# hangxu0304/DeepReduce

Measured on NVIDIA H100. Metric: ResNet-50 images/sec (whole job, device-timed, max over ranks), higher is better.
Workload: dtype bf16

## Files before the change

deepreduce_b200/ops/csrc/binding.cpp:

```cpp
#include <ATen/cuda/CUDAContext.h>
#include <c10/cuda/CUDAGuard.h>
#include <c10/cuda/CUDAStream.h>
#include <torch/extension.h>

#include <condition_variable>
#include <deque>
#include <mutex>
#include <thread>

#include "ops.h"

namespace py = pybind11;
using dr::EngineParams;

#define CHECK_CUDA_T(x) TORCH_CHECK((x).is_cuda() && (x).is_contiguous(), #x " must be a contiguous CUDA tensor")

static cudaStream_t cur_stream() { return at::cuda::getCurrentCUDAStream().stream(); }

static void check_last(const char* what) {
  cudaError_t e = cudaGetLastError();
  TORCH_CHECK(e == cudaSuccess, what, ": ", cudaGetErrorString(e));
}

static torch::Tensor bloom_insert(torch::Tensor idx, int64_t k, int64_t m_bits, int64_t seed) {
  CHECK_CUDA_T(idx);
  TORCH_CHECK(idx.scalar_type() == torch::kInt64, "idx must be int64");
  c10::cuda::CUDAGuard g(idx.device());
  const int64_t n_words = (m_bits + 31) / 32;
  auto words = torch::zeros({n_words}, idx.options().dtype(torch::kInt32));
  dr::launch_bloom_insert(idx.data_ptr<int64_t>(), idx.numel(), (uint32_t*)words.data_ptr<int32_t>(), (uint32_t)k,
                          (uint32_t)m_bits, (uint32_t)seed, cur_stream());
  check_last("bloom_insert");
  return words;
}

static torch::Tensor bloom_select(torch::Tensor words, int64_t d, int64_t limit, int64_t k, int64_t m_bits, int64_t seed) {
  CHECK_CUDA_T(words);
  c10::cuda::CUDAGuard g(words.device());
  const int64_t n_tiles = (d + dr::kTile - 1) / dr::kTile;
// ... 171 lines not shown
  const int64_t total = ones_incl[n_pairs - 1].item<int64_t>();
  auto out = torch::empty({total}, o64);
  dr::launch_rle_expand(ones_excl.data_ptr<int64_t>(), run_start.data_ptr<int64_t>(), n_pairs, total, out.data_ptr<int64_t>(),
                        cur_stream());
  check_last("rle_indices");
  return out;
}

static torch::Tensor u8_to_nhwc_norm(torch::Tensor in, std::vector<double> mean, std::vector<double> stdv) {
  CHECK_CUDA_T(in);
  TORCH_CHECK(in.scalar_type() == torch::kUInt8 && in.size(-1) == 3, "expect uint8 [...,3] NHWC");
  c10::cuda::CUDAGuard g(in.device());
  auto out = torch::empty(in.sizes(), in.options().dtype(torch::kBFloat16));
  float m[3] = {(float)mean[0], (float)mean[1], (float)mean[2]};
  float s[3] = {(float)(1.0 / stdv[0]), (float)(1.0 / stdv[1]), (float)(1.0 / stdv[2])};
  dr::launch_u8_to_nhwc_norm(in.data_ptr<uint8_t>(), out.data_ptr(), in.numel() / 3, m, s, cur_stream());
  check_last("u8_to_nhwc_norm");
  return out;
}

namespace at::native {
struct Var;
template <typename scalar_t, typename VarTransform>
void batch_norm_stats_channels_last_cuda_template(const at::Tensor& out_mean, const at::Tensor& out_invstd,
                                                   const at::Tensor& input, double epsilon);
}

static void check_bn_input(const torch::Tensor& x) {
  TORCH_CHECK(x.is_cuda() && x.scalar_type() == torch::kBFloat16 && x.dim() == 4 && x.stride(1) == 1 &&
                  x.is_contiguous(at::MemoryFormat::ChannelsLast),
              "bn: x must be a channels_last bf16 CUDA tensor");
  TORCH_CHECK(x.size(1) % 8 == 0 && x.size(1) <= 8192, "bn: channels must be a multiple of 8, at most 8192");
  TORCH_CHECK(x.numel() < std::numeric_limits<int32_t>::max(), "bn: tensor too large for 32-bit indexing");
}

static void check_chan(const torch::Tensor& t, int64_t C, const char* what) {
  TORCH_CHECK(t.is_cuda() && t.scalar_type() == torch::kFloat32 && t.is_contiguous() && t.numel() == C, "bn: ", what,
              " must be a contiguous float32 CUDA tensor of C elements");
}

static std::vector<torch::Tensor> bn_stats(torch::Tensor x, torch::Tensor running_mean, torch::Tensor running_var,
                                           double momentum, double eps, bool torch_kernel) {
  check_bn_input(x);
  const int64_t C = x.size(1);
  check_chan(running_mean, C, "running_mean");
  check_chan(running_var, C, "running_var");
  const int64_t N = x.numel() / C;
  TORCH_CHECK(N > 1, "bn: expected more than 1 value per channel when training");
  c10::cuda::CUDAGuard g(x.device());
  auto opts = x.options().dtype(torch::kFloat32);
  auto mean = torch::empty({C}, opts), invstd = torch::empty({C}, opts);
  const float bessel = static_cast<float>(static_cast<double>(N) / static_cast<double>(N - 1));
  int block_y = 0, grid_y = 0;
  dr::bn_row_tree(N, (int)C, &block_y, &grid_y);
  cudaError_t e;
  if (!torch_kernel && (int64_t)block_y * grid_y <= N) {
    auto staging = grid_y > 1 ? torch::empty({(2 * C + 1) * grid_y}, opts) : torch::Tensor();
    const dr::BnStats s{x.data_ptr(), mean.data_ptr<float>(), invstd.data_ptr<float>(), running_mean.data_ptr<float>(),
                        running_var.data_ptr<float>(), grid_y > 1 ? staging.data_ptr<float>() : nullptr,
                        (float)momentum, bessel, (float)eps};
    e = dr::launch_bn_stats(s, N, (int)C, cur_stream());
  } else {
    at::native::batch_norm_stats_channels_last_cuda_template<c10::BFloat16, at::native::Var>(mean, invstd, x, eps);
    e = dr::launch_bn_update_stats(mean.data_ptr<float>(), invstd.data_ptr<float>(), running_mean.data_ptr<float>(),
                                   running_var.data_ptr<float>(), (int)C, (float)momentum, bessel, (float)eps,
                                   cur_stream());
// ... 64 lines not shown

static std::vector<torch::Tensor> bn_backward(int64_t mode, torch::Tensor go, torch::Tensor mask, torch::Tensor x,
                                              std::vector<torch::Tensor> p, c10::optional<torch::Tensor> z,
                                              std::vector<torch::Tensor> pz, c10::optional<torch::Tensor> go2) {
  TORCH_CHECK(mode >= 0 && mode <= 3, "bn_backward: mode must be 0, 1, 2 or 3");
  TORCH_CHECK(!go2.has_value() || mode != 0, "bn_backward: mode 0 takes no go2");
  check_bn_input(x);
  const int64_t C = x.size(1), rows = x.numel() / C;
  dr::PoolGeom pg{(int)x.size(2), (int)x.size(3), (int)((x.size(2) - 1) / 2 + 1), (int)((x.size(3) - 1) / 2 + 1)};
  const std::vector<int64_t> go_shape =
      mode == 3 ? std::vector<int64_t>{x.size(0), C, pg.Ho, pg.Wo} : x.sizes().vec();
  for (const torch::Tensor* t : {&go, go2.has_value() ? &*go2 : &go})
    TORCH_CHECK(t->sizes() == go_shape && t->scalar_type() == torch::kBFloat16 && t->device() == x.device() &&
                    t->is_contiguous(at::MemoryFormat::ChannelsLast),
                "bn_backward: go and go2 must be channels_last bf16 tensors on x's device, of x's shape (mode 3: the "
                "pooled shape)");
  const int64_t mask_numel = mode == 3 ? go.numel() : rows * (C / 8);
  TORCH_CHECK(mask.is_cuda() && mask.scalar_type() == torch::kUInt8 && mask.is_contiguous() &&
                  mask.numel() == mask_numel && mask.device() == x.device(),
              "bn_backward: mask must be bn_apply's mask (mode 3: bn_apply_pool's codes) for x");
  c10::cuda::CUDAGuard guard(x.device());
  int block_y = 0, grid_y = 0;
  dr::bn_row_tree(rows, (int)C, &block_y, &grid_y);
  TORCH_CHECK((int64_t)block_y * grid_y <= rows, "bn_backward: reduction tree wider than the rows");
  const int n_sums = mode == 2 ? 3 : 2;
  auto f32 = x.options().dtype(torch::kFloat32);
  auto sums = torch::empty({n_sums, C}, f32);
  auto staging = grid_y > 1 ? torch::empty({n_sums, grid_y, C}, f32) : torch::Tensor();
  auto dx = torch::empty_like(x), dw = torch::empty({C}, f32), db = torch::empty({C}, f32);
  dr::BnBwd b{};
  b.go = go.data_ptr(); b.go2 = go2.has_value() ? go2->data_ptr() : nullptr; b.mask = mask.data_ptr<uint8_t>(); b.x = x.data_ptr();
  b.px = bn_bwd_params(p, C);
  b.dx = dx.data_ptr(); b.sums = sums.data_ptr<float>(); b.staging = grid_y > 1 ? staging.data_ptr<float>() : nullptr;
  b.dw = dw.data_ptr<float>(); b.db = db.data_ptr<float>();
  b.pool = pg;
  std::vector<torch::Tensor> res{dx, dw, db};
  torch::Tensor g;
  if (mode == 1 || mode == 3) {
    g = torch::empty_like(x);
    b.g = g.data_ptr();
    if (mode == 1) res.push_back(g);
  } else if (mode == 2) {
    TORCH_CHECK(z.has_value(), "bn_backward: mode 2 needs z");
    check_like_x(*z, x, "z");
    b.z = z->data_ptr();
    b.pz = bn_bwd_params(pz, C);
    auto dz = torch::empty_like(x), dwz = torch::empty({C}, f32), dbz = torch::empty({C}, f32);
    b.dz = dz.data_ptr(); b.dwz = dwz.data_ptr<float>(); b.dbz = dbz.data_ptr<float>();
    res.insert(res.end(), {dz, dwz, dbz});
  }
  cudaError_t e = dr::launch_bn_backward((int)mode, b, rows, (int)C, cur_stream());
  TORCH_CHECK(e == cudaSuccess, "bn_backward: ", cudaGetErrorString(e));
  return res;
}

struct Engine {
  EngineParams P{};
  int grid = 0;
  int grid_cap = 0;
  int blocks_per_sm = 2;
  int dyn_smem = 64 * 1024;
  int device = 0;

  Engine(int64_t tensors, int64_t tiles, int64_t n_tensors, int64_t n_tiles, int64_t slot_words,
         int64_t payload_words, int64_t grad, int64_t resid, int64_t hist, int64_t hist_total, int64_t sel,
         int64_t tile_count, int64_t barrier, int64_t status, std::vector<int64_t> arenas, int rank, int world) {
// ... 256 lines not shown
```

deepreduce_b200/ops/csrc/bn.cu:

```cuda
#include <cuda_bf16.h>

#include <algorithm>

#include "common.cuh"
#include "ops.h"

namespace dr {

namespace {

constexpr int kVec = 8;
constexpr int kApplyThreads = 256;
constexpr int kReduceThreads = 128;

struct ChanParams {
  float m[kVec], inv[kVec], w[kVec], b[kVec];
};

__device__ __forceinline__ void load8(const float* __restrict__ p, float* d) {
  const float4 a = __ldg(reinterpret_cast<const float4*>(p));
  const float4 b = __ldg(reinterpret_cast<const float4*>(p) + 1);
  d[0] = a.x; d[1] = a.y; d[2] = a.z; d[3] = a.w;
  d[4] = b.x; d[5] = b.y; d[6] = b.z; d[7] = b.w;
}
// ... 196 lines not shown
                                                                     const uint8_t* __restrict__ codes,
                                                                     __nv_bfloat16* __restrict__ g, PoolGeom pg,
                                                                     int64_t rows, int C) {
  const int groups = C / kVec;
  const int rows_per_cta = blockDim.x / groups;
  const int rsub = threadIdx.x / groups;
  if (rsub >= rows_per_cta) return;
  const int c = (threadIdx.x % groups) * kVec;
  const int64_t step = (int64_t)gridDim.x * rows_per_cta;
#pragma unroll 2
  for (int64_t r = (int64_t)blockIdx.x * rows_per_cta + rsub; r < rows; r += step) {
    PoolGather q;
    pool_gather_codes(q, codes, pg, (int)r, C, c, true);
    pool_gather_grads<kTwo>(q, gp, gp2, pg, C);
    uint4 v;
    unsigned bits;
    pool_gather_resolve(q, v, bits);
    __nv_bfloat16* hv = reinterpret_cast<__nv_bfloat16*>(&v);
#pragma unroll
    for (int i = 0; i < kVec; ++i)
      if (!((bits >> i) & 1u)) hv[i] = __float2bfloat16_rn(0.f);
    *reinterpret_cast<uint4*>(g + r * C + c) = v;
  }
}

struct RowTree {
  int block_y, grid_y;
  __host__ __device__ int S() const { return block_y * grid_y; }
  __host__ __device__ int loops(int rows) const { return 1 + (rows - 1) / (S() * kLoads); }
  static constexpr int kLoads = 4;
};

constexpr int kStatsThreads = 256;

__device__ __forceinline__ void welford_update(float x, float inv, float valid, float& mean, float& m2n) {
  const float d0 = __fsub_rn(x, mean);
  mean = __fmaf_rn(d0, inv, mean);
  const float d1 = __fsub_rn(x, mean);
  m2n = __fmaf_rn(__fmul_rn(d0, d1), valid, m2n);
}

template <int kN, bool kFuseNew>
__device__ __forceinline__ void welford_merge(int& n, float* mean, float* m2n, int n_new, const float* mean_new,
                                              const float* m2n_new) {
  const float fn = (float)n, fn_new = (float)n_new;
  const float factor = __frcp_rn((float)max(1, n + n_new));
#pragma unroll
  for (int i = 0; i < kN; ++i) {
    const float d = __fsub_rn(mean[i], mean_new[i]);
    const float s = kFuseNew ? __fmaf_rn(mean_new[i], fn_new, __fmul_rn(mean[i], fn))
                             : __fmaf_rn(mean[i], fn, __fmul_rn(mean_new[i], fn_new));
    mean[i] = __fmul_rn(s, factor);
    const float u = __fmul_rn(__fmul_rn(__fmul_rn(d, d), fn_new), fn);
    m2n[i] = __fadd_rn(m2n[i], __fmaf_rn(u, factor, m2n_new[i]));
  }
  n += n_new;
}

template <int kN>
struct WelfordSlots {
  float* mean; float* m2n; int* count;
  __device__ WelfordSlots(float* sh, int slots)
      : mean(sh), m2n(sh + slots * kN), count(reinterpret_cast<int*>(sh + 2 * slots * kN)) {}
  __device__ void put(int s, int n, const float* m, const float* q) const {
#pragma unroll
    for (int i = 0; i < kN; ++i) { mean[s * kN + i] = m[i]; m2n[s * kN + i] = q[i]; }
// ... 5 lines not shown
#pragma unroll
    for (int i = 0; i < kN; ++i) { mn[i] = mean[s * kN + i]; qn[i] = m2n[s * kN + i]; }
    welford_merge<kN, kFuseNew>(n, m, q, count[s], mn, qn);
  }
  static size_t bytes(int slots) { return (size_t)slots * (2 * kN * sizeof(float) + sizeof(int)); }
};

template <int kN>
__device__ __forceinline__ void welford_tree_over_y(const WelfordSlots<kN>& sl, bool part, int y, int block_y, int base,
                                                    int stride, int& n, float* mean, float* m2n) {
  for (int off = block_y / 2; off > 0; off >>= 1) {
    if (part && y < 2 * off) sl.put(base + y * stride, n, mean, m2n);
    __syncthreads();
    if (part && y < off) sl.template merge_from<false>(base + (y + off) * stride, n, mean, m2n);
    __syncthreads();
  }
}

struct StatsOut {
  float* mean; float* invstd; float* running_mean; float* running_var;
  float* st_mean; float* st_m2n; int* st_count;
  float momentum, bessel, eps;
};

__device__ __forceinline__ void stats_store(const StatsOut& o, int c, int n, float mean, float m2n) {
  const float var = __fdiv_rn(m2n, (float)n);
  const float keep = __fsub_rn(1.f, o.momentum);
  o.mean[c] = mean;
  o.invstd[c] = rsqrtf(__fadd_rn(var, o.eps));
  o.running_mean[c] = __fmaf_rn(mean, o.momentum, __fmul_rn(o.running_mean[c], keep));
  o.running_var[c] = __fmaf_rn(__fmul_rn(var, o.bessel), o.momentum, __fmul_rn(o.running_var[c], keep));
}

__global__ void __launch_bounds__(kStatsThreads) bn_stats_kernel(const __nv_bfloat16* __restrict__ x, StatsOut o,
                                                                 RowTree t, int rows, int C) {
  constexpr int L = RowTree::kLoads;
  constexpr int kAhead = 4;
  extern __shared__ float sh[];
  const int gpc = blockDim.x / (L * t.block_y);
  const int g = threadIdx.x % gpc, j = (threadIdx.x / gpc) % L, y = threadIdx.x / (gpc * L);
  const int group = blockIdx.x * gpc + g;
  const bool live = group * kVec < C;
  const int c = live ? group * kVec : 0;
  const int S = t.S();
  const int n_loops = t.loops(rows);
  const int r0 = blockIdx.y * t.block_y + y + j * S;
  const int rstep = L * S;
  float mean[kVec], m2n[kVec];
#pragma unroll
  for (int i = 0; i < kVec; ++i) mean[i] = m2n[i] = 0.f;
  int n = 0;
  auto load = [&](uint4* b, int i0) {
#pragma unroll
    for (int u = 0; u < kAhead; ++u) {
      const int r = r0 + (i0 + u) * rstep;
      b[u] = live && i0 + u < n_loops && r < rows ? *reinterpret_cast<const uint4*>(x + (size_t)r * C + c) : uint4{};
    }
  };
  uint4 cur[kAhead];
  load(cur, 0);
  for (int i0 = 0; i0 < n_loops; i0 += kAhead) {
    uint4 nxt[kAhead];
    load(nxt, i0 + kAhead);
#pragma unroll
    for (int u = 0; u < kAhead; ++u) {
      const int i = i0 + u;
      if (i >= n_loops) break;
      const bool valid = r0 + i * rstep < rows;
      const float inv = valid ? __frcp_rn((float)(i + 1)) : 0.f;
      const float fv = valid ? 1.f : 0.f;
      n += valid;
      const __nv_bfloat16* hx = reinterpret_cast<const __nv_bfloat16*>(&cur[u]);
#pragma unroll
      for (int k = 0; k < kVec; ++k) welford_update(__bfloat162float(hx[k]), inv, fv, mean[k], m2n[k]);
    }
#pragma unroll
    for (int u = 0; u < kAhead; ++u) cur[u] = nxt[u];
  }
  const WelfordSlots<kVec> sl(sh, blockDim.x);
  sl.put(threadIdx.x, n, mean, m2n);
  __syncthreads();
  if (j == 0) {
#pragma unroll
    for (int a = 1; a < L; ++a) sl.merge_from<true>(threadIdx.x + a * gpc, n, mean, m2n);
  }
  __syncthreads();
  welford_tree_over_y<kVec>(sl, j == 0, y, t.block_y, g, gpc * L, n, mean, m2n);
  if (j != 0 || y != 0 || !live) return;
  if (t.grid_y == 1) {
#pragma unroll
    for (int i = 0; i < kVec; ++i) stats_store(o, c + i, n, mean[i], m2n[i]);
    return;
  }
#pragma unroll
  for (int i = 0; i < kVec; ++i) {
    o.st_mean[(size_t)blockIdx.y * C + c + i] = mean[i];
    o.st_m2n[(size_t)blockIdx.y * C + c + i] = m2n[i];
  }
  if (group == 0) o.st_count[blockIdx.y] = n;
}

__global__ void bn_stats_finalize_kernel(StatsOut o, RowTree t, int C) {
  extern __shared__ float sh[];
  const int cols = blockDim.x / t.block_y;
  const int col = threadIdx.x % cols, y = threadIdx.x / cols;
  const int c = blockIdx.x * cols + col;
  int n = 0;
  float mean = 0.f, m2n = 0.f;
  if (c < C)
    for (int b = y; b < t.grid_y; b += t.block_y) {
      const float mb = o.st_mean[(size_t)b * C + c], qb = o.st_m2n[(size_t)b * C + c];
      welford_merge<1, false>(n, &mean, &m2n, o.st_count[b], &mb, &qb);
    }
  const WelfordSlots<1> sl(sh, blockDim.x);
  welford_tree_over_y<1>(sl, true, y, t.block_y, col, cols, n, &mean, &m2n);
  if (y == 0 && c < C) stats_store(o, c, n, mean, m2n);
}


template <int kN>
__device__ __forceinline__ void tree_over_y(float* v, float* sh, int y, int n, int col, int width) {
  for (int off = n / 2; off > 0; off >>= 1) {
#pragma unroll
    for (int i = 0; i < kN; ++i) sh[y * width + col + i] = v[i];
    __syncthreads();
    if (y < off) {
#pragma unroll
      for (int i = 0; i < kN; ++i) v[i] = __fadd_rn(v[i], sh[(y + off) * width + col + i]);
    }
    __syncthreads();
  }
}

struct BwdOut {
  float* sums;
  float* dw; float* db; float* dwz; float* dbz;
  float* staging;
};

__device__ __forceinline__ void bwd_store(const BwdOut& o, int k, int c, int C, float v, const float* invstd,
                                         const float* invstd_z) {
  o.sums[k * C + c] = v;
  if (k == 0) {
    o.db[c] = v;
    if (o.dbz) o.dbz[c] = v;
  } else if (k == 1) {
    o.dw[c] = __fmul_rn(v, invstd[c]);
  } else {
    o.dwz[c] = __fmul_rn(v, invstd_z[c]);
  }
}

__device__ __forceinline__ float masked(__nv_bfloat16 go, unsigned bit) { return bit ? __bfloat162float(go) : 0.f; }

template <int kMode, bool kTwo>
__global__ void __launch_bounds__(kReduceThreads) bn_bwd_reduce_kernel(const __nv_bfloat16* __restrict__ go,
                                                                       const __nv_bfloat16* __restrict__ go2,
                                                                       const uint8_t* __restrict__ mask,
                                                                       const __nv_bfloat16* __restrict__ x,
                                                                       const float* __restrict__ mean,
                                                                       const float* __restrict__ invstd,
                                                                       const __nv_bfloat16* __restrict__ z,
                                                                       const float* __restrict__ mean_z,
                                                                       const float* __restrict__ invstd_z,
                                                                       __nv_bfloat16* __restrict__ g_out, BwdOut o,
                                                                       RowTree t, int rows, int C) {
  constexpr int kSums = kMode == 2 ? 3 : 2;
  constexpr int L = RowTree::kLoads;
  extern __shared__ float sh[];
  const int gpc = blockDim.x / t.block_y;
// ... 71 lines not shown
    if (kAhead) cur = nxt;
    r += L * S;
  }
#pragma unroll
  for (int k = 0; k < kSums; ++k) {
#pragma unroll
    for (int i = 0; i < kVec; ++i)
#pragma unroll
      for (int j = 1; j < L; ++j) acc[k][0][i] = __fadd_rn(acc[k][0][i], acc[k][j][i]);
    tree_over_y<kVec>(acc[k][0], sh, y, t.block_y, tg * kVec, gpc * kVec);
  }
  if (y != 0 || !live) return;
#pragma unroll
  for (int k = 0; k < kSums; ++k)
#pragma unroll
    for (int i = 0; i < kVec; ++i) {
      if (t.grid_y > 1) o.staging[((size_t)k * t.grid_y + blockIdx.y) * C + c + i] = acc[k][0][i];
      else bwd_store(o, k, c + i, C, acc[k][0][i], invstd, invstd_z);
    }
}

__global__ void bn_bwd_finalize_kernel(BwdOut o, RowTree t, int n_sums, int C, const float* __restrict__ invstd,
                                       const float* __restrict__ invstd_z) {
  extern __shared__ float sh[];
  const int cols = blockDim.x / t.block_y;
  const int col = threadIdx.x % cols, y = threadIdx.x / cols;
  const int c = blockIdx.x * cols + col;
  for (int k = 0; k < n_sums; ++k) {
    float v = 0.f;
    if (c < C)
      for (int b = y; b < t.grid_y; b += t.block_y) v = __fadd_rn(v, o.staging[((size_t)k * t.grid_y + b) * C + c]);
    tree_over_y<1>(&v, sh, y, t.block_y, col, cols);
    if (y == 0 && c < C) bwd_store(o, k, c, C, v, invstd, invstd_z);
  }
}

struct ElemtChan {
  float m[kVec], f1[kVec], f2[kVec], sdy[kVec];
};

__device__ __forceinline__ void elemt_params(const float* mean, const float* invstd, const float* w, const float* sdy,
                                             const float* sxmu, float norm, int c, ElemtChan& p) {
  float inv[kVec], ww[kVec], sx[kVec];
  load8(mean + c, p.m);
  load8(invstd + c, inv);
  load8(w + c, ww);
  load8(sdy + c, p.sdy);
  load8(sxmu + c, sx);
#pragma unroll
  for (int i = 0; i < kVec; ++i) {
    p.f1[i] = __fmul_rn(__fmul_rn(__fmul_rn(inv[i], inv[i]), sx[i]), norm);
    p.f2[i] = __fmul_rn(ww[i], inv[i]);
  }
}

__device__ __forceinline__ __nv_bfloat16 elemt(float g, float x, const ElemtChan& p, int i, float norm) {
  const float a = __fmaf_rn(-p.sdy[i], norm, g);
  return __float2bfloat16_rn(__fmul_rn(__fmaf_rn(-p.f1[i], __fsub_rn(x, p.m[i]), a), p.f2[i]));
}

struct ElemtArgs {
  const float *mean, *invstd, *weight, *sums;
  const float *mean_z, *invstd_z, *weight_z;
};

template <int kMode, bool kTwo>
// ... 65 lines not shown
  const int64_t cap = (int64_t)(per_sm > 0 ? per_sm : 1) * sm_count();
  grid = (int)(g > cap ? cap : g);
  return cudaSuccess;
}

template <int kMode>
cudaError_t launch_apply(const void* x, const BnParams& px, const void* z, const BnParams& pz, void* out, void* mask,
                         int64_t rows, int C, cudaStream_t st) {
  if (rows == 0) return cudaSuccess;
  int grid = 0, threads = 0;
  cudaError_t e = rows_grid(bn_apply_kernel<kMode>, rows, C, grid, threads);
  if (e != cudaSuccess) return e;
  count_launch();
  bn_apply_kernel<kMode><<<grid, threads, 0, st>>>(reinterpret_cast<const __nv_bfloat16*>(x), px,
                                                   reinterpret_cast<const __nv_bfloat16*>(z), pz,
                                                   reinterpret_cast<__nv_bfloat16*>(out),
                                                   reinterpret_cast<uint8_t*>(mask), rows, C);
  return cudaGetLastError();
}

int last_pow2(unsigned n) {
  n |= n >> 1; n |= n >> 2; n |= n >> 4; n |= n >> 8; n |= n >> 16;
  return std::max<int>(1, (int)(n - (n >> 1)));
}

RowTree row_tree(int rows, int C) {
  const int block_x = std::min(last_pow2((unsigned)C), 32);
  const int block_y = std::min(last_pow2((unsigned)((rows + 15) / 16)), 512 / block_x);
  int grid_y = std::min((rows + block_y * 16 - 1) / (block_y * 16), 128);
  if (grid_y < 8) grid_y = 1;
  return {block_y, grid_y};
}

template <int kMode, bool kTwo>
cudaError_t launch_bwd_reduce(const BnBwd& b, const RowTree& t, const BwdOut& o, int rows, int C, cudaStream_t st) {
  const int groups = C / kVec;
  const int gpc = std::min(groups, std::max(1, kReduceThreads / t.block_y));
  const dim3 grid((groups + gpc - 1) / gpc, t.grid_y);
  const int threads = gpc * t.block_y;
  count_launch();
  bn_bwd_reduce_kernel<kMode, kTwo><<<grid, threads, threads * kVec * sizeof(float), st>>>(
      reinterpret_cast<const __nv_bfloat16*>(b.go), reinterpret_cast<const __nv_bfloat16*>(b.go2), b.mask,
      reinterpret_cast<const __nv_bfloat16*>(b.x), b.px.mean, b.px.invstd, reinterpret_cast<const __nv_bfloat16*>(b.z),
      b.pz.mean, b.pz.invstd, reinterpret_cast<__nv_bfloat16*>(b.g), o, t, rows, C);
  return cudaGetLastError();
}

template <int kMode, bool kTwo>
cudaError_t launch_bwd_elemt(const BnBwd& b, const ElemtArgs& a, int64_t rows, int C, cudaStream_t st) {
  int grid = 0, threads = 0;
  cudaError_t e = rows_grid(bn_bwd_elemt_kernel<kMode, kTwo>, rows, C, grid, threads);
  if (e != cudaSuccess) return e;
  const float norm = (float)(1.0 / (double)rows);
  count_launch();
  bn_bwd_elemt_kernel<kMode, kTwo><<<grid, threads, 0, st>>>(
      reinterpret_cast<const __nv_bfloat16*>(kMode == 1 || kMode == 3 ? b.g : b.go),
      reinterpret_cast<const __nv_bfloat16*>(b.go2), b.mask, reinterpret_cast<const __nv_bfloat16*>(b.x),
      reinterpret_cast<const __nv_bfloat16*>(b.z), a, reinterpret_cast<__nv_bfloat16*>(b.dx),
      reinterpret_cast<__nv_bfloat16*>(b.dz), norm, rows, C);
  return cudaGetLastError();
}

template <int kMode, bool kTwo>
cudaError_t launch_backward(const BnBwd& b, int64_t rows64, int C, cudaStream_t st) {
  const int rows = (int)rows64;
  const RowTree t = row_tree(rows, C);
  const BwdOut o{b.sums, b.dw, b.db, b.dwz, b.dbz, b.staging};
  cudaError_t e;
  if (kMode == 3) {
    int grid = 0, threads = 0;
    e = rows_grid(bn_pool_grad_kernel<kTwo>, rows64, C, grid, threads);
    if (e != cudaSuccess) return e;
    count_launch();
    bn_pool_grad_kernel<kTwo><<<grid, threads, 0, st>>>(reinterpret_cast<const __nv_bfloat16*>(b.go),
                                                        reinterpret_cast<const __nv_bfloat16*>(b.go2), b.mask,
                                                        reinterpret_cast<__nv_bfloat16*>(b.g), b.pool, rows64, C);
    e = cudaGetLastError();
    if (e != cudaSuccess) return e;
  }
  BnBwd bb = b;
  if (kMode == 3) bb.go = b.g;
  e = launch_bwd_reduce<kMode, kTwo && kMode != 3>(bb, t, o, rows, C, st);
  if (e != cudaSuccess) return e;
  if (t.grid_y > 1) {
    const int cols = std::max(1, 512 / t.block_y);
    const int threads = cols * t.block_y;
    count_launch();
    bn_bwd_finalize_kernel<<<(C + cols - 1) / cols, threads, threads * sizeof(float), st>>>(
        o, t, kMode == 2 ? 3 : 2, C, b.px.invstd, b.pz.invstd);
    e = cudaGetLastError();
    if (e != cudaSuccess) return e;
  }
  const ElemtArgs a{b.px.mean, b.px.invstd, b.px.weight, b.sums, b.pz.mean, b.pz.invstd, b.pz.weight};
  return launch_bwd_elemt<kMode, kTwo && kMode == 2>(b, a, rows64, C, st);
}

cudaError_t launch_stats(const BnStats& s, int rows, int C, cudaStream_t st) {
  const RowTree t = row_tree(rows, C);
  const int grid_y = t.grid_y;
  const StatsOut o{s.mean, s.invstd, s.running_mean, s.running_var,
                   s.staging, s.staging + (size_t)grid_y * C, reinterpret_cast<int*>(s.staging + 2 * (size_t)grid_y * C),
                   s.momentum, s.bessel, s.eps};
  const int groups = C / kVec;
  const int gpc = std::min(groups, std::max(1, kStatsThreads / (RowTree::kLoads * t.block_y)));
  const int threads = gpc * RowTree::kLoads * t.block_y;
  count_launch();
  bn_stats_kernel<<<dim3((groups + gpc - 1) / gpc, grid_y), threads, WelfordSlots<kVec>::bytes(threads), st>>>(
      reinterpret_cast<const __nv_bfloat16*>(s.x), o, t, rows, C);
  cudaError_t e = cudaGetLastError();
  if (e != cudaSuccess || grid_y == 1) return e;
  const int cols = std::max(1, 512 / t.block_y);
  const int fthreads = cols * t.block_y;
  count_launch();
  bn_stats_finalize_kernel<<<(C + cols - 1) / cols, fthreads, WelfordSlots<1>::bytes(fthreads), st>>>(o, t, C);
  return cudaGetLastError();
}

}

void bn_row_tree(int64_t rows, int C, int* block_y, int* grid_y) {
  const RowTree t = row_tree((int)rows, C);
  *block_y = t.block_y;
  *grid_y = t.grid_y;
}

cudaError_t launch_bn_backward(int mode, const BnBwd& b, int64_t rows, int C, cudaStream_t st) {
  if (rows == 0) return cudaSuccess;
  const bool two = b.go2 != nullptr;
  switch (mode) {
    case 0: return two ? cudaErrorInvalidValue : launch_backward<0, false>(b, rows, C, st);
    case 1: return two ? launch_backward<1, true>(b, rows, C, st) : launch_backward<1, false>(b, rows, C, st);
    case 2: return two ? launch_backward<2, true>(b, rows, C, st) : launch_backward<2, false>(b, rows, C, st);
    case 3: return two ? launch_backward<3, true>(b, rows, C, st) : launch_backward<3, false>(b, rows, C, st);
    default: return cudaErrorInvalidValue;
  }
}

cudaError_t launch_bn_stats(const BnStats& s, int64_t rows, int C, cudaStream_t st) {
  if (rows == 0) return cudaSuccess;
  return launch_stats(s, (int)rows, C, st);
}
// ... 35 lines not shown
```

deepreduce_b200/ops/csrc/ops.h:

```cpp
#pragma once
#include <cuda_runtime.h>
#include <stdint.h>

#include "plan.h"

namespace dr {

int engine_max_grid(int blocks_per_sm, int dyn_smem_bytes);
cudaError_t engine_launch(const EngineParams& P, int grid, int blocks_per_sm, int dyn_smem_bytes, cudaStream_t stream);
void count_launch(int n);
long long launch_count();

void launch_bloom_insert(const int64_t* idx, int64_t n, uint32_t* filter, uint32_t n_hash, uint32_t m_bits,
                         uint32_t seed, cudaStream_t st);
void launch_bloom_count(const uint32_t* filter, uint32_t d, uint32_t n_hash, uint32_t m_bits, uint32_t seed,
                        uint32_t* tile_counts, uint32_t* tile_excl, cudaStream_t st);
void launch_bloom_emit(const uint32_t* filter, uint32_t d, uint32_t n_hash, uint32_t m_bits, uint32_t seed,
                       const uint32_t* tile_excl, int64_t* out, uint32_t limit, cudaStream_t st);
void launch_qsgd_encode(const float* v, int64_t K, int bucket, int q, uint32_t seed, void* lvl, bool i16, float* norms,
                        cudaStream_t st);
void launch_qsgd_decode(const void* lvl, bool i16, const float* norms, int64_t K, int bucket, int q, float* out,
                        cudaStream_t st);
void launch_pack_bits(const int64_t* vals, int64_t n, int bits, uint32_t* out, int64_t n_words, cudaStream_t st);
void launch_unpack_bits(const uint32_t* in, int64_t n_words, int64_t n, int bits, int64_t* out, cudaStream_t st);
// ... 15 lines not shown
                       cudaStream_t st);

struct ArenaHandle { unsigned char bytes[64]; };
void* arena_alloc(size_t bytes);
void arena_free(void* p);
ArenaHandle arena_export(void* p);
void* arena_import(const ArenaHandle& h);
void arena_close(void* p);
int arena_enable_peer_access(const int* devices, int n);
void launch_u8_to_nhwc_norm(const uint8_t* in, void* out_bf16, int64_t n_pix, const float* mean, const float* inv_std,
                            cudaStream_t st);

struct BnParams { const float* mean; const float* invstd; const float* weight; const float* bias; };
void bn_row_tree(int64_t rows, int C, int* block_y, int* grid_y);
struct BnStats {
  const void* x;
  float* mean; float* invstd; float* running_mean; float* running_var;
  float* staging;
  float momentum, bessel, eps;
};
cudaError_t launch_bn_stats(const BnStats& s, int64_t rows, int C, cudaStream_t st);
cudaError_t launch_bn_update_stats(const float* mean, float* var_invstd, float* running_mean, float* running_var, int C,
                                   float momentum, float bessel, float eps, cudaStream_t st);
cudaError_t launch_bn_apply(int mode, const void* x, const BnParams& px, const void* z, const BnParams& pz, void* out,
                            void* mask, int64_t rows, int C, cudaStream_t st);
struct PoolGeom { int H, W, Ho, Wo; };
cudaError_t launch_bn_apply_pool(const void* x, const BnParams& px, void* out, void* codes, int N, const PoolGeom& pg,
                                 int C, cudaStream_t st);
struct BnBwd {
  const void* go; const void* go2; const uint8_t* mask; const void* x; const void* z;
  BnParams px, pz;
  void* dx; void* dz; void* g;
  float* sums; float* staging; float* dw; float* db; float* dwz; float* dbz;
  PoolGeom pool;
};
cudaError_t launch_bn_backward(int mode, const BnBwd& b, int64_t rows, int C, cudaStream_t st);

}
```

Measured before the change: 5184.

## Fuse BN backward cross-block reduction via last-block tickets; add wide-channel stats variant

For small row-tree sizes, BN backward's reduce kernel now finishes the cross-block sum itself: each block writes partials to staging, and the last block to arrive (tracked with per-stream atomic ticket counters) sums them and stores the final dw/db. This removes a separate finalize launch. BN stats gets a templated variant for wide layouts that keeps several Welford accumulators per thread in registers, so it uses fewer threads and skips a shared-memory merge. The trade-offs are a threadfence plus atomic per block, persistent ticket buffers, and more register pressure.

```diff
diff --git a/deepreduce_b200/ops/csrc/binding.cpp b/deepreduce_b200/ops/csrc/binding.cpp
--- a/deepreduce_b200/ops/csrc/binding.cpp
+++ b/deepreduce_b200/ops/csrc/binding.cpp
@@ -5,6 +5,7 @@
 
 #include <condition_variable>
 #include <deque>
+#include <map>
 #include <mutex>
 #include <thread>
 
@@ -242,6 +243,19 @@
               "bn: x must be a channels_last bf16 CUDA tensor");
   TORCH_CHECK(x.size(1) % 8 == 0 && x.size(1) <= 8192, "bn: channels must be a multiple of 8, at most 8192");
   TORCH_CHECK(x.numel() < std::numeric_limits<int32_t>::max(), "bn: tensor too large for 32-bit indexing");
+}
+
+static int* bn_tickets(cudaStream_t st) {
+  static std::mutex mu;
+  static auto* bufs = new std::map<std::pair<int, cudaStream_t>, int*>();
+  const int dev = c10::cuda::current_device();
+  std::lock_guard<std::mutex> l(mu);
+  int*& p = (*bufs)[{dev, st}];
+  if (p == nullptr) {
+    C10_CUDA_CHECK(cudaMalloc(&p, dr::kBnTickets * sizeof(int)));
+    C10_CUDA_CHECK(cudaMemsetAsync(p, 0, dr::kBnTickets * sizeof(int), st));
+  }
+  return p;
 }
 
 static void check_chan(const torch::Tensor& t, int64_t C, const char* what) {
@@ -372,6 +386,7 @@
   b.go = go.data_ptr(); b.go2 = go2.has_value() ? go2->data_ptr() : nullptr; b.mask = mask.data_ptr<uint8_t>(); b.x = x.data_ptr();
   b.px = bn_bwd_params(p, C);
   b.dx = dx.data_ptr(); b.sums = sums.data_ptr<float>(); b.staging = grid_y > 1 ? staging.data_ptr<float>() : nullptr;
+  b.tickets = grid_y > 1 ? bn_tickets(cur_stream()) : nullptr;
   b.dw = dw.data_ptr<float>(); b.db = db.data_ptr<float>();
   b.pool = pg;
   std::vector<torch::Tensor> res{dx, dw, db};
diff --git a/deepreduce_b200/ops/csrc/bn.cu b/deepreduce_b200/ops/csrc/bn.cu
--- a/deepreduce_b200/ops/csrc/bn.cu
+++ b/deepreduce_b200/ops/csrc/bn.cu
@@ -252,6 +252,7 @@
 };
 
 constexpr int kStatsThreads = 256;
+constexpr int kStatsWideThreads = 128;
 
 __device__ __forceinline__ void welford_update(float x, float inv, float valid, float& mean, float& m2n) {
   const float d0 = __fsub_rn(x, mean);
@@ -323,72 +324,93 @@
   o.running_var[c] = __fmaf_rn(__fmul_rn(var, o.bessel), o.momentum, __fmul_rn(o.running_var[c], keep));
 }
 
-__global__ void __launch_bounds__(kStatsThreads) bn_stats_kernel(const __nv_bfloat16* __restrict__ x, StatsOut o,
-                                                                 RowTree t, int rows, int C) {
+template <int kAcc>
+__global__ void __launch_bounds__(kAcc == 1 ? kStatsThreads : kStatsWideThreads, kAcc == 1 ? 1 : 4)
+    bn_stats_kernel(const __nv_bfloat16* __restrict__ x, StatsOut o, RowTree t, int rows, int C) {
   constexpr int L = RowTree::kLoads;
-  constexpr int kAhead = 4;
+  constexpr int P = L / kAcc;
+  constexpr int kAhead = L / kAcc;
   extern __shared__ float sh[];
-  const int gpc = blockDim.x / (L * t.block_y);
-  const int g = threadIdx.x % gpc, j = (threadIdx.x / gpc) % L, y = threadIdx.x / (gpc * L);
+  const int gpc = blockDim.x / (P * t.block_y);
+  const int g = threadIdx.x % gpc, p = (threadIdx.x / gpc) % P, y = threadIdx.x / (gpc * P);
   const int group = blockIdx.x * gpc + g;
   const bool live = group * kVec < C;
   const int c = live ? group * kVec : 0;
   const int S = t.S();
   const int n_loops = t.loops(rows);
-  const int r0 = blockIdx.y * t.block_y + y + j * S;
+  const int r0 = blockIdx.y * t.block_y + y + p * kAcc * S;
   const int rstep = L * S;
-  float mean[kVec], m2n[kVec];
-#pragma unroll
-  for (int i = 0; i < kVec; ++i) mean[i] = m2n[i] = 0.f;
-  int n = 0;
-  auto load = [&](uint4* b, int i0) {
-#pragma unroll
-    for (int u = 0; u < kAhead; ++u) {
-      const int r = r0 + (i0 + u) * rstep;
-      b[u] = live && i0 + u < n_loops && r < rows ? *reinterpret_cast<const uint4*>(x + (size_t)r * C + c) : uint4{};
-    }
+  float mean[kAcc][kVec], m2n[kAcc][kVec];
+  int n[kAcc];
+#pragma unroll
+  for (int a = 0; a < kAcc; ++a) {
+    n[a] = 0;
+#pragma unroll
+    for (int i = 0; i < kVec; ++i) mean[a][i] = m2n[a][i] = 0.f;
+  }
+  auto load = [&](uint4 (*b)[kAcc], int i0) {
+#pragma unroll
+    for (int u = 0; u < kAhead; ++u)
+#pragma unroll
+      for (int a = 0; a < kAcc; ++a) {
+        const int r = r0 + a * S + (i0 + u) * rstep;
+        b[u][a] = live && i0 + u < n_loops && r < rows ? *reinterpret_cast<const uint4*>(x + (size_t)r * C + c)
+                                                       : uint4{};
+      }
   };
-  uint4 cur[kAhead];
+  uint4 cur[kAhead][kAcc];
   load(cur, 0);
   for (int i0 = 0; i0 < n_loops; i0 += kAhead) {
-    uint4 nxt[kAhead];
+    uint4 nxt[kAhead][kAcc];
     load(nxt, i0 + kAhead);
 #pragma unroll
     for (int u = 0; u < kAhead; ++u) {
       const int i = i0 + u;
       if (i >= n_loops) break;
-      const bool valid = r0 + i * rstep < rows;
-      const float inv = valid ? __frcp_rn((float)(i + 1)) : 0.f;
-      const float fv = valid ? 1.f : 0.f;
-      n += valid;
-      const __nv_bfloat16* hx = reinterpret_cast<const __nv_bfloat16*>(&cur[u]);
-#pragma unroll
-      for (int k = 0; k < kVec; ++k) welford_update(__bfloat162float(hx[k]), inv, fv, mean[k], m2n[k]);
-    }
-#pragma unroll
-    for (int u = 0; u < kAhead; ++u) cur[u] = nxt[u];
+      const float rc = __frcp_rn((float)(i + 1));
+#pragma unroll
+      for (int a = 0; a < kAcc; ++a) {
+        const bool valid = r0 + a * S + i * rstep < rows;
+        const float inv = valid ? rc : 0.f;
+        const float fv = valid ? 1.f : 0.f;
+        n[a] += valid;
+        const __nv_bfloat16* hx = reinterpret_cast<const __nv_bfloat16*>(&cur[u][a]);
+#pragma unroll
+        for (int k = 0; k < kVec; ++k) welford_update(__bfloat162float(hx[k]), inv, fv, mean[a][k], m2n[a][k]);
+      }
+    }
+#pragma unroll
+    for (int u = 0; u < kAhead; ++u)
+#pragma unroll
+      for (int a = 0; a < kAcc; ++a) cur[u][a] = nxt[u][a];
   }
   const WelfordSlots<kVec> sl(sh, blockDim.x);
-  sl.put(threadIdx.x, n, mean, m2n);
-  __syncthreads();
-  if (j == 0) {
-#pragma unroll
-    for (int a = 1; a < L; ++a) sl.merge_from<true>(threadIdx.x + a * gpc, n, mean, m2n);
-  }
-  __syncthreads();
-  welford_tree_over_y<kVec>(sl, j == 0, y, t.block_y, g, gpc * L, n, mean, m2n);
-  if (j != 0 || y != 0 || !live) return;
+  int& n0 = n[0];
+  if (kAcc == 1) {
+    sl.put(threadIdx.x, n0, mean[0], m2n[0]);
+    __syncthreads();
+    if (p == 0) {
+#pragma unroll
+      for (int a = 1; a < L; ++a) sl.merge_from<true>(threadIdx.x + a * gpc, n0, mean[0], m2n[0]);
+    }
+    __syncthreads();
+  } else {
+#pragma unroll
+    for (int a = 1; a < kAcc; ++a) welford_merge<kVec, true>(n0, mean[0], m2n[0], n[a], mean[a], m2n[a]);
+  }
+  welford_tree_over_y<kVec>(sl, p == 0, y, t.block_y, g, gpc * P, n0, mean[0], m2n[0]);
+  if (p != 0 || y != 0 || !live) return;
   if (t.grid_y == 1) {
 #pragma unroll
-    for (int i = 0; i < kVec; ++i) stats_store(o, c + i, n, mean[i], m2n[i]);
+    for (int i = 0; i < kVec; ++i) stats_store(o, c + i, n0, mean[0][i], m2n[0][i]);
     return;
   }
 #pragma unroll
   for (int i = 0; i < kVec; ++i) {
-    o.st_mean[(size_t)blockIdx.y * C + c + i] = mean[i];
-    o.st_m2n[(size_t)blockIdx.y * C + c + i] = m2n[i];
-  }
-  if (group == 0) o.st_count[blockIdx.y] = n;
+    o.st_mean[(size_t)blockIdx.y * C + c + i] = mean[0][i];
+    o.st_m2n[(size_t)blockIdx.y * C + c + i] = m2n[0][i];
+  }
+  if (group == 0) o.st_count[blockIdx.y] = n0;
 }
 
 __global__ void bn_stats_finalize_kernel(StatsOut o, RowTree t, int C) {
@@ -427,6 +449,7 @@
   float* sums;
   float* dw; float* db; float* dwz; float* dbz;
   float* staging;
+  int* tickets;
 };
 
 __device__ __forceinline__ void bwd_store(const BwdOut& o, int k, int c, int C, float v, const float* invstd,
@@ -564,6 +587,170 @@
       for (int b = y; b < t.grid_y; b += t.block_y) v = __fadd_rn(v, o.staging[((size_t)k * t.grid_y + b) * C + c]);
     tree_over_y<1>(&v, sh, y, t.block_y, col, cols);
     if (y == 0 && c < C) bwd_store(o, k, c, C, v, invstd, invstd_z);
+  }
+}
+
+constexpr int kSplitThreads = 512;
+constexpr int kFinPer = kVec / RowTree::kLoads;
+
+template <int kN>
+__device__ __forceinline__ void sum_tree_over_y(float* sh, int slots, bool part, int y, int block_y, int base,
+                                                int stride, float* v) {
+  for (int off = block_y / 2; off > 0; off >>= 1) {
+    if (part && y < 2 * off) {
+#pragma unroll
+      for (int i = 0; i < kN; ++i) sh[i * slots + base + y * stride] = v[i];
+    }
+    __syncthreads();
+    if (part && y < off) {
+#pragma unroll
+      for (int i = 0; i < kN; ++i) v[i] = __fadd_rn(v[i], sh[i * slots + base + (y + off) * stride]);
+    }
+    __syncthreads();
+  }
+}
+
+__device__ __forceinline__ bool last_block(int* tickets, int grid_y) {
+  __shared__ int last;
+  __threadfence();
+  __syncthreads();
+  if (threadIdx.x == 0) {
+    last = atomicAdd(tickets + blockIdx.x, 1) == grid_y - 1;
+    if (last) tickets[blockIdx.x] = 0;
+  }
+  __syncthreads();
+  return last;
+}
+
+template <int kMode, bool kTwo>
+__global__ void __launch_bounds__(kSplitThreads, 1) bn_bwd_reduce_split_kernel(const __nv_bfloat16* __restrict__ go,
+                                                                               const __nv_bfloat16* __restrict__ go2,
+                                                                               const uint8_t* __restrict__ mask,
+                                                                               const __nv_bfloat16* __restrict__ x,
+                                                                               const float* __restrict__ mean,
+                                                                               const float* __restrict__ invstd,
+                                                                               const __nv_bfloat16* __restrict__ z,
+                                                                               const float* __restrict__ mean_z,
+                                                                               const float* __restrict__ invstd_z,
+                                                                               __nv_bfloat16* __restrict__ g_out,
+                                                                               BwdOut o, RowTree t, int rows, int C) {
+  constexpr int kSums = kMode == 2 ? 3 : 2;
+  constexpr int kN = kSums * kVec;
+  constexpr int L = RowTree::kLoads;
+  constexpr int kAhead = kMode == 2 || kTwo ? 2 : 4;
+  extern __shared__ float sh[];
+  const int gpc = blockDim.x / (L * t.block_y);
+  const int g = threadIdx.x % gpc, j = (threadIdx.x / gpc) % L, y = threadIdx.x / (gpc * L);
+  const int group = blockIdx.x * gpc + g;
+  const bool live = group * kVec < C;
+  const int c = live ? group * kVec : 0;
+  const int S = t.S();
+  const int n_loops = t.loops(rows);
+  const int r0 = blockIdx.y * t.block_y + y + j * S;
+  const int rstep = L * S;
+  float m[kVec], mz[kVec];
+#pragma unroll
+  for (int i = 0; i < kVec; ++i) {
+    m[i] = mean[c + i];
+    mz[i] = kMode == 2 ? mean_z[c + i] : 0.f;
+  }
+  float acc[kN];
+#pragma unroll
+  for (int q = 0; q < kN; ++q) acc[q] = 0.f;
+  const int mgroups = C / kVec;
+  struct Row {
+    uint4 g, g2, x, z;
+    unsigned m;
+  };
+  auto load = [&](Row* b, int i0) {
+#pragma unroll
+    for (int u = 0; u < kAhead; ++u) {
+      const int r = r0 + (i0 + u) * rstep;
+      if (live && i0 + u < n_loops && r < rows) {
+        const int off = r * C + c;
+        b[u].g = *reinterpret_cast<const uint4*>(go + off);
+        if (kTwo) b[u].g2 = *reinterpret_cast<const uint4*>(go2 + off);
+        b[u].x = *reinterpret_cast<const uint4*>(x + off);
+        if (kMode == 2) b[u].z = *reinterpret_cast<const uint4*>(z + off);
+        b[u].m = kMode == 3 ? 0u : mask[r * mgroups + group];
+      } else {
+        b[u].g = uint4{}; b[u].g2 = uint4{}; b[u].x = uint4{}; b[u].z = uint4{}; b[u].m = 0;
+      }
+    }
+  };
+  Row cur[kAhead];
+  load(cur, 0);
+  for (int i0 = 0; i0 < n_loops; i0 += kAhead) {
+    if (kTwo) {
+#pragma unroll
+      for (int u = 0; u < kAhead; ++u) cur[u].g = add_bf16x8(cur[u].g, cur[u].g2);
+    }
+    Row nxt[kAhead];
+    load(nxt, i0 + kAhead);
+#pragma unroll
+    for (int u = 0; u < kAhead; ++u) {
+      const int i = i0 + u;
+      if (i >= n_loops) break;
+      const int r = r0 + i * rstep;
+      const __nv_bfloat16* hg = reinterpret_cast<const __nv_bfloat16*>(&cur[u].g);
+      const __nv_bfloat16* hx = reinterpret_cast<const __nv_bfloat16*>(&cur[u].x);
+      const __nv_bfloat16* hz = reinterpret_cast<const __nv_bfloat16*>(&cur[u].z);
+      uint4 vo;
+      __nv_bfloat16* ho = reinterpret_cast<__nv_bfloat16*>(&vo);
+#pragma unroll
+      for (int k = 0; k < kVec; ++k) {
+        const unsigned bit = (cur[u].m >> k) & 1u;
+        const float gk = kMode == 3 ? __bfloat162float(hg[k]) : masked(hg[k], bit);
+        if (kMode == 1) ho[k] = bit ? hg[k] : __float2bfloat16_rn(0.f);
+        acc[k] = __fadd_rn(acc[k], gk);
+        acc[kVec + k] = __fmaf_rn(__fsub_rn(__bfloat162float(hx[k]), m[k]), gk, acc[kVec + k]);
+        if (kMode == 2) acc[2 * kVec + k] = __fmaf_rn(__fsub_rn(__bfloat162float(hz[k]), mz[k]), gk, acc[2 * kVec + k]);
+      }
+      if (kMode == 1 && live && r < rows) *reinterpret_cast<uint4*>(g_out + r * C + c) = vo;
+    }
+#pragma unroll
+    for (int u = 0; u < kAhead; ++u) cur[u] = nxt[u];
+  }
+  const int slots = blockDim.x;
+#pragma unroll
+  for (int q = 0; q < kN; ++q) sh[q * slots + threadIdx.x] = acc[q];
+  __syncthreads();
+  if (j == 0) {
+#pragma unroll
+    for (int a = 1; a < L; ++a)
+#pragma unroll
+      for (int q = 0; q < kN; ++q) acc[q] = __fadd_rn(acc[q], sh[q * slots + threadIdx.x + a * gpc]);
+  }
+  __syncthreads();
+  sum_tree_over_y<kN>(sh, slots, j == 0, y, t.block_y, g, gpc * L, acc);
+  const bool head = j == 0 && y == 0 && live;
+  if (t.grid_y == 1) {
+    if (head) {
+#pragma unroll
+      for (int q = 0; q < kN; ++q) bwd_store(o, q / kVec, c + q % kVec, C, acc[q], invstd, invstd_z);
+    }
+    return;
+  }
+  if (head) {
+#pragma unroll
+    for (int q = 0; q < kN; ++q) o.staging[((size_t)(q / kVec) * t.grid_y + blockIdx.y) * C + c + q % kVec] = acc[q];
+  }
+  if (!last_block(o.tickets, t.grid_y)) return;
+  constexpr int kF = kSums * kFinPer;
+  const int cf = c + j * kFinPer;
+  float v[kF];
+#pragma unroll
+  for (int q = 0; q < kF; ++q) v[q] = 0.f;
+  if (live)
+    for (int b = y; b < t.grid_y; b += t.block_y) {
+#pragma unroll
+      for (int q = 0; q < kF; ++q)
+        v[q] = __fadd_rn(v[q], __ldcg(o.staging + ((size_t)(q / kFinPer) * t.grid_y + b) * C + cf + q % kFinPer));
+    }
+  sum_tree_over_y<kF>(sh, slots, true, y, t.block_y, threadIdx.x % (gpc * L), gpc * L, v);
+  if (y == 0 && live) {
+#pragma unroll
+    for (int q = 0; q < kF; ++q) bwd_store(o, q / kFinPer, cf + q % kFinPer, C, v[q], invstd, invstd_z);
   }
 }
 
@@ -695,6 +882,28 @@
   return {block_y, grid_y};
 }
 
+constexpr int64_t kSplitMaxThreads = 16 * 1024;
+
+template <int kMode, bool kTwo>
+cudaError_t launch_bwd_reduce_split(const BnBwd& b, const RowTree& t, const BwdOut& o, int rows, int C,
+                                   cudaStream_t st) {
+  constexpr int kSums = kMode == 2 ? 3 : 2;
+  constexpr int kSmemMax = kSplitThreads * kSums * kVec * sizeof(float);
+  static const cudaError_t attr = cudaFuncSetAttribute(bn_bwd_reduce_split_kernel<kMode, kTwo>,
+                                                       cudaFuncAttributeMaxDynamicSharedMemorySize, kSmemMax);
+  if (attr != cudaSuccess) return attr;
+  const int groups = C / kVec;
+  const int gpc = std::min(groups, std::max(1, kSplitThreads / (RowTree::kLoads * t.block_y)));
+  const dim3 grid((groups + gpc - 1) / gpc, t.grid_y);
+  const int threads = gpc * RowTree::kLoads * t.block_y;
+  count_launch();
+  bn_bwd_reduce_split_kernel<kMode, kTwo><<<grid, threads, threads * kSums * kVec * sizeof(float), st>>>(
+      reinterpret_cast<const __nv_bfloat16*>(b.go), reinterpret_cast<const __nv_bfloat16*>(b.go2), b.mask,
+      reinterpret_cast<const __nv_bfloat16*>(b.x), b.px.mean, b.px.invstd, reinterpret_cast<const __nv_bfloat16*>(b.z),
+      b.pz.mean, b.pz.invstd, reinterpret_cast<__nv_bfloat16*>(b.g), o, t, rows, C);
+  return cudaGetLastError();
+}
+
 template <int kMode, bool kTwo>
 cudaError_t launch_bwd_reduce(const BnBwd& b, const RowTree& t, const BwdOut& o, int rows, int C, cudaStream_t st) {
   const int groups = C / kVec;
@@ -728,7 +937,7 @@
 cudaError_t launch_backward(const BnBwd& b, int64_t rows64, int C, cudaStream_t st) {
   const int rows = (int)rows64;
   const RowTree t = row_tree(rows, C);
-  const BwdOut o{b.sums, b.dw, b.db, b.dwz, b.dbz, b.staging};
+  const BwdOut o{b.sums, b.dw, b.db, b.dwz, b.dbz, b.staging, b.tickets};
   cudaError_t e;
   if (kMode == 3) {
     int grid = 0, threads = 0;
@@ -743,9 +952,11 @@
   }
   BnBwd bb = b;
   if (kMode == 3) bb.go = b.g;
-  e = launch_bwd_reduce<kMode, kTwo && kMode != 3>(bb, t, o, rows, C, st);
+  const bool split = (int64_t)t.S() * (C / kVec) <= kSplitMaxThreads;
+  e = split ? launch_bwd_reduce_split<kMode, kTwo && kMode != 3>(bb, t, o, rows, C, st)
+            : launch_bwd_reduce<kMode, kTwo && kMode != 3>(bb, t, o, rows, C, st);
   if (e != cudaSuccess) return e;
-  if (t.grid_y > 1) {
+  if (!split && t.grid_y > 1) {
     const int cols = std::max(1, 512 / t.block_y);
     const int threads = cols * t.block_y;
     count_launch();
@@ -765,11 +976,19 @@
                    s.staging, s.staging + (size_t)grid_y * C, reinterpret_cast<int*>(s.staging + 2 * (size_t)grid_y * C),
                    s.momentum, s.bessel, s.eps};
   const int groups = C / kVec;
-  const int gpc = std::min(groups, std::max(1, kStatsThreads / (RowTree::kLoads * t.block_y)));
-  const int threads = gpc * RowTree::kLoads * t.block_y;
+  const bool narrow = (int64_t)t.S() * groups <= kSplitMaxThreads;
+  const int per_virtual = narrow ? RowTree::kLoads : 1;
+  const int cap = narrow ? kStatsThreads : kStatsWideThreads;
+  const int gpc = std::min(groups, std::max(1, cap / (per_virtual * t.block_y)));
+  const int threads = gpc * per_virtual * t.block_y;
+  const dim3 grid((groups + gpc - 1) / gpc, grid_y);
   count_launch();
-  bn_stats_kernel<<<dim3((groups + gpc - 1) / gpc, grid_y), threads, WelfordSlots<kVec>::bytes(threads), st>>>(
-      reinterpret_cast<const __nv_bfloat16*>(s.x), o, t, rows, C);
+  if (narrow)
+    bn_stats_kernel<1><<<grid, threads, WelfordSlots<kVec>::bytes(threads), st>>>(
+        reinterpret_cast<const __nv_bfloat16*>(s.x), o, t, rows, C);
+  else
+    bn_stats_kernel<RowTree::kLoads><<<grid, threads, WelfordSlots<kVec>::bytes(threads), st>>>(
+        reinterpret_cast<const __nv_bfloat16*>(s.x), o, t, rows, C);
   cudaError_t e = cudaGetLastError();
   if (e != cudaSuccess || grid_y == 1) return e;
   const int cols = std::max(1, 512 / t.block_y);
diff --git a/deepreduce_b200/ops/csrc/ops.h b/deepreduce_b200/ops/csrc/ops.h
--- a/deepreduce_b200/ops/csrc/ops.h
+++ b/deepreduce_b200/ops/csrc/ops.h
@@ -71,8 +71,10 @@
   BnParams px, pz;
   void* dx; void* dz; void* g;
   float* sums; float* staging; float* dw; float* db; float* dwz; float* dbz;
+  int* tickets;
   PoolGeom pool;
 };
+constexpr int kBnTickets = 8192 / 8;
 cudaError_t launch_bn_backward(int mode, const BnBwd& b, int64_t rows, int C, cudaStream_t st);
 
 }
```

Measured after the change: 5297, median of 6. 2.2% higher.
